# harskish/ganspace

Hardware: NVIDIA H100
Metric: latent samples/sec into PCA (StyleGAN2-ffhq W, N=1e6) (higher is better)
Workload: dtype f32

## Files before the change

ganspace_b200/_native.py:

```python
from __future__ import annotations

import contextlib
import ctypes as C
import os
from pathlib import Path

import torch

_LIB_PATH = Path(__file__).resolve().parent / "libganspace_b200.so"
_lib = None

_P, _I, _L, _Z, _D, _F = C.c_void_p, C.c_int, C.c_int64, C.c_size_t, C.c_double, C.c_float
SIGNATURES = {
    "gsb_abi_version": (_I, []),
    "gsb_last_error": (C.c_char_p, []),
    "gsb_legacy_normal_f32": (_I, [_P, _I, _L, _P, _L, _P]),
    "gsb_legacy_truncnorm_f32": (_I, [_P, _I, _L, _D, _D, _F, _P, _L, _P]),
    "gsb_mt19937_raw_u32": (_I, [_P, _I, _L, _P, _L, _P]),
    "gsb_mt19937_jump_polys": (_I, [_L, _I, _P]),
    "gsb_mt19937_jump_state_host": (_I, [C.c_uint32, _P, _P]),
    "gsb_legacy_normal_split_step_words": (_L, [_L, _I]),
    "gsb_legacy_normal_split_workspace_bytes": (_Z, [_I, _L, _I]),
    "gsb_legacy_normal_f32_split": (_I, [_P, _I, _L, _P, _L, _I, _P, _P, _Z, _P]),
    "gsb_legacy_normal_split_status": (_I, [_P, _I, _L, _I, _P, _P]),
# ... 140 lines not shown
    def add_rows(self, name, n):
        self.rows[name] = self.rows.get(name, 0) + int(n)

    def count(self, n):
        self.launches += n

    class _Sec:
        def __init__(self, outer, name):
            self.o, self.name = outer, name

        def __enter__(self):
            if self.o.timing:
                self.e0 = torch.cuda.Event(enable_timing=True)
                self.e1 = torch.cuda.Event(enable_timing=True)
                self.e0.record(torch.cuda.current_stream())

        def __exit__(self, *a):
            if self.o.timing:
                self.e1.record(torch.cuda.current_stream())
                self.o._events.setdefault(self.name, []).append((self.e0, self.e1))
            self.o.mark(self.name + " done")

    def section(self, name):
        return self._Sec(self, name)

    def section_ms(self):
        torch.cuda.synchronize()
        return {k: (sum(a.elapsed_time(b) for a, b in v), len(v)) for k, v in self._events.items()}


instrument = _Instrument()

SECTION_KERNELS = {
    "mapping": "mapping MLP: pixelnorm_split + 8 x mapping_layer_tc_kernel (wgmma, fp16 hi/lo x3)",
    "linear": "gen_z linear: mapping_layer_tc_kernel (wgmma, fp16 hi/lo x3, bias epilogue, TMA store) for n >= 128",
    "synthesis": "StyledConv chain: tap-GEMM tc_gemm_plain (wgmma) + gather/scatter/blur epilogues",
}


def kernel_name(section: str) -> str:
    if section == "mapping" and os.environ.get("GANSPACE_B200_MAPPING", MAPPING_DEFAULT) == "simt":
        return "mapping MLP: pixelnorm + 8 x sgemm_tn_bias_act_kernel (fp32 FMA)"
    return SECTION_KERNELS.get(section, section)


class _Scratch:

    def __init__(self):
        self._bufs = {}

    def get(self, key, nbytes: int, device) -> torch.Tensor:
        k = (key, str(device))
        buf = self._bufs.get(k)
        if buf is None or buf.numel() < nbytes:
            buf = torch.empty(max(int(nbytes), 256), dtype=torch.uint8, device=device)
            self._bufs[k] = buf
        return buf

    def clear(self):
        self._bufs.clear()


scratch = _Scratch()


_jump_polys = {}


def jump_polys(n_per_stream: int, parts: int, device) -> torch.Tensor:
    import numpy as np
    lib = load()
    step = int(lib.gsb_legacy_normal_split_step_words(int(n_per_stream), int(parts)))
    key = (step, parts - 1)
    if key not in _jump_polys:
        table = np.zeros((parts - 1, 624), np.uint32)
# ... 92 lines not shown
        self.n_layers, self.dim = int(weight.shape[0]), int(weight.shape[1])
        assert weight.shape == (self.n_layers, self.dim, self.dim) and bias.shape == (self.n_layers, self.dim)
        self.device = dev
        self.packed = torch.empty(lib.gsb_mapping_packed_bytes(self.n_layers, self.dim), dtype=torch.uint8, device=dev)
        w = weight.detach().to(dev, torch.float32).contiguous()
        b = bias.detach().to(dev, torch.float32).contiguous()
        with torch.cuda.device(dev):
            _check(lib.gsb_mapping_pack(_ptr(w), _ptr(b), self.n_layers, self.dim, float(lr_mul),
                                        _ptr(self.packed), _stream()), "gsb_mapping_pack")

    def check(self):
        flags = C.c_uint(0)
        with torch.cuda.device(self.device):
            _check(load().gsb_mapping_status(_ptr(self.packed), self.n_layers, self.dim, C.byref(flags)),
                   "gsb_mapping_status")
        if flags.value & 1:
            raise NativeError("mapping network: an activation exceeded fp16 range in the tensor-core path; "
                              "results are invalid (set GANSPACE_B200_MAPPING=simt)")

    def forward(self, z: torch.Tensor, out: torch.Tensor = None, pixelnorm: bool = True,
                force_simt: bool = None, leave_free_sms: int = 0) -> torch.Tensor:
        lib = load()
        if force_simt is None:
            force_simt = os.environ.get("GANSPACE_B200_MAPPING", MAPPING_DEFAULT) == "simt"
        assert z.is_cuda and z.dtype == torch.float32 and z.shape[-1] == self.dim
        z2 = z.reshape(-1, self.dim)
        if not z2.is_contiguous():
            z2 = z2.contiguous()
        n = z2.shape[0]
        if out is None:
            out = torch.empty_like(z2)
        ws_bytes = lib.gsb_mapping_workspace_bytes(n, self.dim)
        ws = scratch.get("mapping", ws_bytes, z.device)
        flags = (1 if pixelnorm else 0) | (2 if force_simt else 0) | ((int(leave_free_sms) & 0xff) << 8)
        with torch.cuda.device(z.device), instrument.section("mapping"):
            _check(lib.gsb_mapping_forward(_ptr(self.packed), self.n_layers, self.dim, _ptr(z2), _ptr(out), n,
                                           flags, _ptr(ws), ws.numel(), _stream()), "gsb_mapping_forward")
        instrument.count(self.n_layers + (1 if pixelnorm else 0))
        instrument.add_rows("mapping", n)
        return out.reshape(z.shape)


def linear(x: torch.Tensor, w: torch.Tensor, bias: torch.Tensor = None, lrelu: bool = False, bounded: bool = False) -> torch.Tensor:
    lib = load()
    assert x.is_cuda and x.dtype == torch.float32 and w.dtype == torch.float32 and x.shape[-1] == w.shape[1]
    x2 = x.reshape(-1, x.shape[-1]).contiguous()
    w = w.contiguous()
    n, K = x2.shape
    N = w.shape[0]
    y = torch.empty((n, N), dtype=torch.float32, device=x.device)
    flags = (1 if lrelu else 0) | (2 if bounded else 0)
    ws = scratch.get("linear", lib.gsb_linear_workspace_bytes(n, N, K, flags), x.device)
    with torch.cuda.device(x.device), instrument.section("linear"):
        _check(lib.gsb_linear_forward(_ptr(x2), _ptr(w), _ptr(bias.contiguous() if bias is not None else None), _ptr(y),
                                      n, N, K, flags, _ptr(ws), ws.numel(), _stream()), "gsb_linear_forward")
    instrument.count(5 if (bounded and n >= 128 and N % 256 == 0 and K % 64 == 0) else 1)
    instrument.add_rows("linear", n)
    return y.reshape(*x.shape[:-1], N)


def mapping_pixelnorm(z: torch.Tensor) -> torch.Tensor:
    lib = load()
    assert z.is_cuda and z.dtype == torch.float32
    dim = z.shape[-1]
    z2 = z.reshape(-1, dim).contiguous()
    out = torch.empty_like(z2)
    ws = scratch.get("mapping", lib.gsb_mapping_workspace_bytes(z2.shape[0], dim), z.device)
    with torch.cuda.device(z.device):
        _check(lib.gsb_mapping_forward(C.c_void_p(0), 0, dim, _ptr(z2), _ptr(out), z2.shape[0], 1, _ptr(ws),
                                       ws.numel(), _stream()), "gsb_mapping_forward")
    return out.reshape(z.shape)
# ... 491 lines not shown
```

ganspace_b200/csrc/mapping.cu:

```cuda
#include "common.cuh"

namespace gsb {

size_t mapping_tc_packed_bytes(int n_layers, int dim);
int mapping_tc_pack(const float *pw, int n_layers, int dim, void *tc_base, cudaStream_t st);
int mapping_forward_tc(const float *pb, void *tc_base, int n_layers, int dim, const float *d_z, float *d_w,
                       int64_t n, bool pixelnorm, void *ws, int leave_free_sms, cudaStream_t st);
size_t mapping_tc_workspace_bytes(int64_t n, int dim);
size_t tc_linear_workspace_bytes(int64_t n, int N, int K);
int tc_linear(const float *x, const float *w, const float *bias, float *y, int64_t n, int N, int K, bool lrelu, void *ws,
              cudaStream_t st);
unsigned *mapping_tc_overflow_flag(void *tc_base, int n_layers, int dim);

static inline size_t simt_packed_bytes(int n_layers, int dim) {
    return align_up(((size_t)n_layers * dim * dim + (size_t)n_layers * dim) * sizeof(float), 256);
}
static inline bool tc_supported(int n_layers, int dim) { return n_layers > 0 && dim % 256 == 0; }

__global__ void mapping_pack_kernel(const float *__restrict__ w, const float *__restrict__ b,
                                    int n_layers, int dim, float scale, float lr_mul,
                                    float *__restrict__ pw, float *__restrict__ pb) {
    int64_t nw = (int64_t)n_layers * dim * dim;
    int64_t nb = (int64_t)n_layers * dim;
    for (int64_t i = blockIdx.x * (int64_t)blockDim.x + threadIdx.x; i < nw + nb;
         i += (int64_t)gridDim.x * blockDim.x) {
        if (i < nw) pw[i] = __fmul_rn(w[i], scale);
        else pb[i - nw] = __fmul_rn(b[i - nw], lr_mul);
    }
}

__global__ void pixelnorm_kernel(const float *__restrict__ x, float *__restrict__ y, int64_t n, int dim) {
    int64_t row = blockIdx.x * (int64_t)(blockDim.x >> 5) + (threadIdx.x >> 5);
    if (row >= n) return;
    const int lane = threadIdx.x & 31;
    const float4 *xr = reinterpret_cast<const float4 *>(x + row * dim);
    float4 *yr = reinterpret_cast<float4 *>(y + row * dim);
    float s = 0.f;
    for (int i = lane; i < dim / 4; i += 32) {
        float4 v = xr[i];
        s += v.x * v.x + v.y * v.y + v.z * v.z + v.w * v.w;
// ... 134 lines not shown
    float scale = (float)((1.0 / sqrt((double)dim)) * (double)lr_mul);
    gsb::mapping_pack_kernel<<<512, 256, 0, (cudaStream_t)stream>>>(d_weight, d_bias, n_layers, dim, scale,
                                                                   lr_mul, pw, pb);
    GSB_CHECK_LAUNCH();
    if (gsb::tc_supported(n_layers, dim)) {
        void *tc_base = reinterpret_cast<char *>(d_packed) + gsb::simt_packed_bytes(n_layers, dim);
        return gsb::mapping_tc_pack(pw, n_layers, dim, tc_base, (cudaStream_t)stream);
    }
    return GSB_OK;
}

extern "C" size_t gsb_mapping_workspace_bytes(int64_t n, int dim) {
    size_t simt = 2 * gsb::align_up((size_t)n * dim * sizeof(float), 256);
    size_t tc = gsb::mapping_tc_workspace_bytes(n, dim);
    return simt > tc ? simt : tc;
}

extern "C" int gsb_mapping_forward(const void *d_packed, int n_layers, int dim, const float *d_z,
                                   float *d_w, int64_t n, int flags, void *d_workspace,
                                   size_t workspace_bytes, gsb_stream_t stream) {
    GSB_CHECK_ARG(d_z && d_w && (d_packed || n_layers == 0), "mapping_forward: null pointer");
    GSB_CHECK_ARG(n_layers >= 0 && dim % 128 == 0, "mapping_forward: dim must be a multiple of 128");
    GSB_CHECK_ARG(n_layers > 0 || (flags & 1), "mapping_forward: nothing to do (n_layers == 0 without PixelNorm)");
    if (n == 0) return GSB_OK;
    if (workspace_bytes < gsb_mapping_workspace_bytes(n, dim) || !d_workspace) {
        gsb::set_error("mapping_forward: workspace too small (%zu < %zu)", workspace_bytes,
                       gsb_mapping_workspace_bytes(n, dim));
        return GSB_ERR_WORKSPACE;
    }
    const float *pw = reinterpret_cast<const float *>(d_packed);
    const float *pb = pw + (size_t)n_layers * dim * dim;
    if (!(flags & 2) && gsb::tc_supported(n_layers, dim)) {
        void *tc_base = reinterpret_cast<char *>(const_cast<void *>(d_packed)) + gsb::simt_packed_bytes(n_layers, dim);
        return gsb::mapping_forward_tc(pb, tc_base, n_layers, dim, d_z, d_w, n, (flags & 1) != 0, d_workspace,
                                       (flags >> 8) & 0xff, (cudaStream_t)stream);
    }
    float *tmp0 = reinterpret_cast<float *>(d_workspace);
    float *tmp1 = reinterpret_cast<float *>(reinterpret_cast<char *>(d_workspace) +
                                            gsb::align_up((size_t)n * dim * sizeof(float), 256));
    return gsb::mapping_forward_simt(pw, pb, n_layers, dim, d_z, d_w, n, (flags & 1) != 0, tmp0, tmp1,
                                     (cudaStream_t)stream);
}

extern "C" int gsb_mapping_status(const void *d_packed, int n_layers, int dim, unsigned *h_flags) {
    GSB_CHECK_ARG(d_packed && h_flags, "mapping_status: null pointer");
    *h_flags = 0;
    if (!gsb::tc_supported(n_layers, dim)) return GSB_OK;
    void *tc_base = reinterpret_cast<char *>(const_cast<void *>(d_packed)) + gsb::simt_packed_bytes(n_layers, dim);
    GSB_CHECK_CUDA(cudaMemcpy(h_flags, gsb::mapping_tc_overflow_flag(tc_base, n_layers, dim), sizeof(unsigned),
                              cudaMemcpyDeviceToHost));
    return GSB_OK;
}

static bool linear_tc_eligible(int64_t n, int N, int K, int flags) {
    return (flags & 2) && n >= 128 && N % 256 == 0 && K % 64 == 0;
}

extern "C" size_t gsb_linear_workspace_bytes(int64_t n, int N, int K, int flags) {
    size_t b = (size_t)N * sizeof(float);
    if (linear_tc_eligible(n, N, K, flags)) {
        size_t t = gsb::tc_linear_workspace_bytes(n, N, K) + gsb::align_up((size_t)N * sizeof(float), 256);
        if (t > b) b = t;
    }
    return b;
}

extern "C" int gsb_linear_forward(const float *d_x, const float *d_w, const float *d_bias, float *d_y, int64_t n,
                                  int N, int K, int flags, void *d_workspace, size_t workspace_bytes,
// ... 27 lines not shown
```

ganspace_b200/csrc/mapping_tc.cu:

```cuda
#include "tc_common.cuh"
#include <stdlib.h>

namespace gsb {

constexpr int TC_BLOCK_M = 128;
constexpr int TC_BLOCK_N = 128;
constexpr int TC_BLOCK_K = 64;
constexpr int TC_STAGES = 3;
constexpr int TC_FRAG_ROWS = 64;
constexpr uint32_t TC_A_BYTES = TC_BLOCK_M * TC_BLOCK_K * 2;
constexpr uint32_t TC_W_BYTES = TC_BLOCK_N * TC_BLOCK_K * 2;
constexpr uint32_t TC_STAGE_BYTES = 2 * TC_A_BYTES + 2 * TC_W_BYTES;
constexpr uint32_t TC_BOX_BYTES = TC_FRAG_ROWS * 128;
constexpr uint32_t TC_STAGING_BYTES = 2 * 2 * TC_BOX_BYTES;
constexpr int TC_THREADS = tc::CONSUMER_THREADS + 128;
constexpr uint32_t TC_SMEM_BYTES = TC_STAGES * TC_STAGE_BYTES + TC_STAGING_BYTES + 64  + 1024 ;
static_assert(TC_SMEM_BYTES <= 232448, "mapping_layer_tc_kernel: shared memory exceeds the H100's 227 KB per block");

struct TcParams {
    const float *bias;
    __half *out_hi;
    __half *out_lo;
    float *out_f32;
    unsigned *overflow;
// ... 128 lines not shown
            int stage = g0 % TC_STAGES, prev = stage;
            uint32_t phase = (uint32_t)(g0 / TC_STAGES) & 1;
            if (i > 0) mbar_wait(&turn_bar[wg], (uint32_t)((i - 1) >> 1) & 1);
            for (int kb = 0; kb < num_k_blocks; ++kb) {
                mbar_wait(&full_bar[stage], phase);
                if (!(p.dbg & 8)) {
                    const uint32_t st = smem_u32(smem + stage * TC_STAGE_BYTES);
                    const uint32_t sw = st + 2 * TC_A_BYTES;
                    const uint64_t d_wh = sw128_kmajor_desc(sw), d_wl = sw128_kmajor_desc(sw + TC_W_BYTES);
                    wgmma_fence();
                    split_kblock_m64n128(acc0, sw128_kmajor_desc(st), sw128_kmajor_desc(st + TC_A_BYTES), d_wh, d_wl, kb > 0);
                    split_kblock_m64n128(acc1, sw128_kmajor_desc(st + TC_A_BYTES / 2),
                                         sw128_kmajor_desc(st + TC_A_BYTES + TC_A_BYTES / 2), d_wh, d_wl, kb > 0);
                    wgmma_commit();
                }
                wgmma_wait_1();
                if (kb > 0 && lane == 0) mbar_arrive(&empty_bar[prev]);
                if (kb == num_k_blocks - 1 && lane == 0) mbar_arrive(&turn_bar[wg ^ 1]);
                prev = stage;
                if (++stage == TC_STAGES) { stage = 0; phase ^= 1; }
            }
            wgmma_wait_all();
            if (lane == 0) mbar_arrive(&empty_bar[prev]);
            store_chunk(acc0, 0, m0, n0, 0);
            store_chunk(acc0, 32, m0, n0, 64);
            store_chunk(acc1, 0, m0 + TC_FRAG_ROWS, n0, 0);
            store_chunk(acc1, 32, m0 + TC_FRAG_ROWS, n0, 64);
        }
        if (ovf) atomicOr(p.overflow, 1u);
        if (storer) asm volatile("cp.async.bulk.wait_group 0;" ::: "memory");
    }
}

__global__ void pixelnorm_split_kernel(const float *__restrict__ x, __half *__restrict__ hi, __half *__restrict__ lo,
                                       int64_t n, int dim, int do_norm, unsigned *overflow) {
    int64_t row = blockIdx.x * (int64_t)(blockDim.x >> 5) + (threadIdx.x >> 5);
    if (row >= n) return;
    const int lane = threadIdx.x & 31;
    const float4 *xr = reinterpret_cast<const float4 *>(x + row * dim);
    float r = 1.f;
    if (do_norm) {
        float s = 0.f;
        for (int i = lane; i < dim / 4; i += 32) {
            float4 v = xr[i];
            s += v.x * v.x + v.y * v.y + v.z * v.z + v.w * v.w;
        }
        s = warp_sum(s);
        r = 1.0f / sqrtf(s / (float)dim + 1e-8f);
    }
    bool ovf = false;
    for (int i = lane; i < dim / 4; i += 32) {
        float4 v = xr[i];
        float f[4] = {v.x * r, v.y * r, v.z * r, v.w * r};
        __half h[4], l[4];
#pragma unroll
        for (int q = 0; q < 4; ++q) {
            h[q] = __float2half_rn(f[q]);
            l[q] = __float2half_rn(f[q] - __half2float(h[q]));
            ovf |= fabsf(f[q]) > 60000.f;
        }
        uint2 ph, pl;
        ph.x = (uint32_t)__half_as_ushort(h[0]) | ((uint32_t)__half_as_ushort(h[1]) << 16);
        ph.y = (uint32_t)__half_as_ushort(h[2]) | ((uint32_t)__half_as_ushort(h[3]) << 16);
        pl.x = (uint32_t)__half_as_ushort(l[0]) | ((uint32_t)__half_as_ushort(l[1]) << 16);
        pl.y = (uint32_t)__half_as_ushort(l[2]) | ((uint32_t)__half_as_ushort(l[3]) << 16);
        reinterpret_cast<uint2 *>(hi + row * dim)[i] = ph;
// ... 24 lines not shown
    }
}

__global__ void absmax_kernel(const float *__restrict__ x, int64_t count, float *__restrict__ out) {
    float m = 0.f;
    for (int64_t i = blockIdx.x * (int64_t)blockDim.x + threadIdx.x; i < count; i += (int64_t)gridDim.x * blockDim.x)
        m = fmaxf(m, fabsf(x[i]));
    for (int o = 16; o > 0; o >>= 1) m = fmaxf(m, __shfl_xor_sync(0xffffffffu, m, o));
    if ((threadIdx.x & 31) == 0) atomicMax(reinterpret_cast<int *>(out), __float_as_int(m));
}

static int make_tmap_f16(CUtensorMap *map, const void *base, uint64_t rows, uint64_t cols, uint32_t box_rows) {
    const uint64_t dims[2] = {cols, rows};
    const uint64_t strides[1] = {cols * 2};
    const uint32_t box[2] = {(uint32_t)TC_BLOCK_K, box_rows};
    return tc_make_tmap_f16(map, base, 2, dims, strides, box);
}

static int make_tmap_f32_out(CUtensorMap *map, const void *base, uint64_t rows, uint64_t cols) {
    TcEncodeTiledFn enc = tc_encode_fn();
    if (!enc) { set_error("cuTensorMapEncodeTiled entry point not available"); return GSB_ERR_CUDA; }
    cuuint64_t gdim[2] = {cols, rows};
    cuuint64_t gstride[1] = {cols * 4};
    cuuint32_t box[2] = {32, (cuuint32_t)TC_FRAG_ROWS};
    cuuint32_t estr[2] = {1, 1};
    CUresult r = enc(map, CU_TENSOR_MAP_DATA_TYPE_FLOAT32, 2, const_cast<void *>(base), gdim, gstride, box, estr,
                     CU_TENSOR_MAP_INTERLEAVE_NONE, CU_TENSOR_MAP_SWIZZLE_128B, CU_TENSOR_MAP_L2_PROMOTION_L2_256B,
                     CU_TENSOR_MAP_FLOAT_OOB_FILL_NONE);
    if (r != CUDA_SUCCESS) { set_error("cuTensorMapEncodeTiled (fp32 output) failed (%d)", (int)r); return GSB_ERR_CUDA; }
    return GSB_OK;
}

size_t mapping_tc_packed_bytes(int n_layers, int dim) {
    return align_up((size_t)n_layers * dim * dim * 2, 256) * 2 + align_up((size_t)3 * n_layers * sizeof(float), 256) + 256;
}

struct TcPackView {
    __half *w_hi, *w_lo;
    float *inv_wscale, *wscale, *absmax;
    unsigned *overflow;
};
static TcPackView tc_pack_view(void *base, int n_layers, int dim) {
    TcPackView v;
    char *p = reinterpret_cast<char *>(base);
    size_t wb = align_up((size_t)n_layers * dim * dim * 2, 256);
    v.w_hi = reinterpret_cast<__half *>(p);
    v.w_lo = reinterpret_cast<__half *>(p + wb);
    v.inv_wscale = reinterpret_cast<float *>(p + 2 * wb);
    v.wscale = v.inv_wscale + n_layers;
    v.absmax = v.wscale + n_layers;
    v.overflow = reinterpret_cast<unsigned *>(p + 2 * wb + align_up((size_t)3 * n_layers * sizeof(float), 256));
    return v;
}

int mapping_tc_pack(const float *pw, int n_layers, int dim, void *tc_base, cudaStream_t st) {
    TcPackView v = tc_pack_view(tc_base, n_layers, dim);
    GSB_CHECK_CUDA(cudaMemsetAsync(v.inv_wscale, 0, (size_t)3 * n_layers * sizeof(float), st));
    GSB_CHECK_CUDA(cudaMemsetAsync(v.overflow, 0, sizeof(unsigned), st));
    const int64_t per = (int64_t)dim * dim;
    for (int l = 0; l < n_layers; ++l) {
        absmax_kernel<<<64, 256, 0, st>>>(pw + l * per, per, v.absmax + l);
        GSB_CHECK_LAUNCH();
        pick_wscale_kernel<<<1, 1, 0, st>>>(v.absmax + l, v.wscale + l, v.inv_wscale + l);
        GSB_CHECK_LAUNCH();
        weight_split_kernel<<<256, 256, 0, st>>>(pw + l * per, per, v.wscale + l, v.w_hi + l * per, v.w_lo + l * per);
        GSB_CHECK_LAUNCH();
    }
    return GSB_OK;
}

static int tc_ensure_attr() {
    static bool attr_set = false;
    if (!attr_set) {
        GSB_CHECK_CUDA(cudaFuncSetAttribute(mapping_layer_tc_kernel, cudaFuncAttributeMaxDynamicSharedMemorySize, (int)TC_SMEM_BYTES));
        attr_set = true;
    }
    return GSB_OK;
}

static int tc_launch_layer(const CUtensorMap &tm_ah, const CUtensorMap &tm_al, const CUtensorMap &tm_wh, const CUtensorMap &tm_wl,
                           TcParams p, int leave_free_sms, cudaStream_t st) {
    CUtensorMap tm_o0, tm_o1;
    if (p.out_f32) {
        if (int r = make_tmap_f32_out(&tm_o0, p.out_f32, (uint64_t)p.M, (uint64_t)p.N_total)) return r;
        tm_o1 = tm_o0;
    } else {
        if (int r = make_tmap_f16(&tm_o0, p.out_hi, (uint64_t)p.M, (uint64_t)p.N_total, TC_FRAG_ROWS)) return r;
        if (int r = make_tmap_f16(&tm_o1, p.out_lo, (uint64_t)p.M, (uint64_t)p.N_total, TC_FRAG_ROWS)) return r;
    }
    const int m_tiles = (p.M + TC_BLOCK_M - 1) / TC_BLOCK_M, n_tiles = (p.N_total + TC_BLOCK_N - 1) / TC_BLOCK_N;
    int avail = num_sms() - leave_free_sms;
    if (avail < 16) avail = 16;
    if (avail > num_sms()) avail = num_sms();
    {
        static int dbg = -1;
        if (dbg < 0) { const char *e = getenv("GANSPACE_B200_MAPPING_DBG"); dbg = e ? atoi(e) : 0; }
        p.dbg = dbg;
    }
    const int64_t units = (int64_t)m_tiles * n_tiles;
    const int grid = units < avail ? (int)units : avail;
    mapping_layer_tc_kernel<<<grid, TC_THREADS, TC_SMEM_BYTES, st>>>(tm_ah, tm_al, tm_wh, tm_wl, tm_o0, tm_o1, p);
    GSB_CHECK_LAUNCH();
    return GSB_OK;
}

int tc_gemm_plain(const __half *a_hi, const __half *a_lo, int64_t M, int K, const __half *w_hi, const __half *w_lo, int N,
                  const float *inv_wscale, float *out, unsigned *overflow, int leave_free_sms, cudaStream_t st) {
    GSB_CHECK_ARG(N % 32 == 0 && N >= 32 && K % 8 == 0 && K >= 8 && M > 0 && M < (1ll << 31),
                  "tc_gemm_plain: need N%%32==0, K%%8==0 (M=%lld N=%d K=%d)", (long long)M, N, K);
    if (int r = tc_ensure_attr()) return r;
    CUtensorMap tm_ah, tm_al, tm_wh, tm_wl;
    if (int r = make_tmap_f16(&tm_ah, a_hi, (uint64_t)M, (uint64_t)K, TC_BLOCK_M)) return r;
    if (int r = make_tmap_f16(&tm_al, a_lo, (uint64_t)M, (uint64_t)K, TC_BLOCK_M)) return r;
    if (int r = make_tmap_f16(&tm_wh, w_hi, (uint64_t)N, (uint64_t)K, TC_BLOCK_N)) return r;
    if (int r = make_tmap_f16(&tm_wl, w_lo, (uint64_t)N, (uint64_t)K, TC_BLOCK_N)) return r;
    TcParams p;
    p.bias = nullptr; p.out_hi = nullptr; p.out_lo = nullptr; p.out_f32 = out; p.overflow = overflow;
    p.inv_wscale = inv_wscale; p.M = (int)M; p.N_total = N; p.K = K; p.mode = 1;
    return tc_launch_layer(tm_ah, tm_al, tm_wh, tm_wl, p, leave_free_sms, st);
}

size_t tc_linear_workspace_bytes(int64_t n, int N, int K) {
    return 2 * align_up((size_t)n * K * 2, 256) + 2 * align_up((size_t)N * K * 2, 256) + 512;
}

int tc_linear(const float *x, const float *w, const float *bias, float *y, int64_t n, int N, int K, bool lrelu, void *ws,
              cudaStream_t st) {
    GSB_CHECK_ARG(N % 256 == 0 && K % TC_BLOCK_K == 0 && n > 0 && n < (1ll << 31) && bias, "tc_linear: need N%%256==0, K%%64==0, bias");
    if (int r = tc_ensure_attr()) return r;
    char *p0 = reinterpret_cast<char *>(ws);
    const size_t xb = align_up((size_t)n * K * 2, 256), wb = align_up((size_t)N * K * 2, 256);
    __half *x_hi = (__half *)p0, *x_lo = (__half *)(p0 + xb), *w_hi = (__half *)(p0 + 2 * xb), *w_lo = (__half *)(p0 + 2 * xb + wb);
    float *scal = (float *)(p0 + 2 * xb + 2 * wb);
    unsigned *overflow = (unsigned *)(p0 + 2 * xb + 2 * wb + 256);
    GSB_CHECK_CUDA(cudaMemsetAsync(scal, 0, 512, st));
    absmax_kernel<<<256, 256, 0, st>>>(w, (int64_t)N * K, scal + 2);
    GSB_CHECK_LAUNCH();
    pick_wscale_kernel<<<1, 1, 0, st>>>(scal + 2, scal + 1, scal);
    GSB_CHECK_LAUNCH();
    weight_split_kernel<<<1024, 256, 0, st>>>(w, (int64_t)N * K, scal + 1, w_hi, w_lo);
    GSB_CHECK_LAUNCH();
    pixelnorm_split_kernel<<<(unsigned)((n + 7) / 8), 256, 0, st>>>(x, x_hi, x_lo, n, K, 0, overflow);
    GSB_CHECK_LAUNCH();
    CUtensorMap tm_ah, tm_al, tm_wh, tm_wl;
    if (int r = make_tmap_f16(&tm_ah, x_hi, (uint64_t)n, (uint64_t)K, TC_BLOCK_M)) return r;
    if (int r = make_tmap_f16(&tm_al, x_lo, (uint64_t)n, (uint64_t)K, TC_BLOCK_M)) return r;
    if (int r = make_tmap_f16(&tm_wh, w_hi, (uint64_t)N, (uint64_t)K, TC_BLOCK_N)) return r;
    if (int r = make_tmap_f16(&tm_wl, w_lo, (uint64_t)N, (uint64_t)K, TC_BLOCK_N)) return r;
    TcParams p;
    p.bias = bias; p.out_hi = nullptr; p.out_lo = nullptr; p.out_f32 = y; p.overflow = overflow;
    p.inv_wscale = scal; p.M = (int)n; p.N_total = N; p.K = K; p.mode = lrelu ? 0 : 2;
    return tc_launch_layer(tm_ah, tm_al, tm_wh, tm_wl, p, 0, st);
}

int mapping_forward_tc(const float *pb, void *tc_base, int n_layers, int dim,
                       const float *d_z, float *d_w, int64_t n, bool pixelnorm, void *ws, int leave_free_sms,
                       cudaStream_t st) {
    GSB_CHECK_ARG(dim % 256 == 0 && dim % TC_BLOCK_K == 0, "mapping_forward_tc: dim must be a multiple of 256");
    GSB_CHECK_ARG(n < (1ll << 31), "mapping_forward_tc: too many rows");
    TcPackView v = tc_pack_view(tc_base, n_layers, dim);
    const size_t buf = align_up((size_t)n * dim * 2, 256);
    __half *a_hi[2] = {reinterpret_cast<__half *>(ws), reinterpret_cast<__half *>((char *)ws + 2 * buf)};
    __half *a_lo[2] = {reinterpret_cast<__half *>((char *)ws + buf), reinterpret_cast<__half *>((char *)ws + 3 * buf)};

    if (int r = tc_ensure_attr()) return r;
    pixelnorm_split_kernel<<<(unsigned)((n + 7) / 8), 256, 0, st>>>(d_z, a_hi[0], a_lo[0], n, dim, pixelnorm ? 1 : 0,
                                                                  v.overflow);
    GSB_CHECK_LAUNCH();
    const int64_t per = (int64_t)dim * dim;
    for (int l = 0; l < n_layers; ++l) {
        const int src = l & 1, dst = src ^ 1;
        CUtensorMap tm_ah, tm_al, tm_wh, tm_wl;
        if (int r = make_tmap_f16(&tm_ah, a_hi[src], (uint64_t)n, dim, TC_BLOCK_M)) return r;
        if (int r = make_tmap_f16(&tm_al, a_lo[src], (uint64_t)n, dim, TC_BLOCK_M)) return r;
        if (int r = make_tmap_f16(&tm_wh, v.w_hi + l * per, dim, dim, TC_BLOCK_N)) return r;
        if (int r = make_tmap_f16(&tm_wl, v.w_lo + l * per, dim, dim, TC_BLOCK_N)) return r;
        TcParams p;
        p.bias = pb + (int64_t)l * dim;
        const bool last = (l == n_layers - 1);
        p.out_hi = last ? nullptr : a_hi[dst];
        p.out_lo = last ? nullptr : a_lo[dst];
        p.out_f32 = last ? d_w : nullptr;
        p.overflow = v.overflow;
        p.inv_wscale = v.inv_wscale + l;
        p.M = (int)n; p.N_total = dim; p.K = dim; p.mode = 0;
        if (int r = tc_launch_layer(tm_ah, tm_al, tm_wh, tm_wl, p, leave_free_sms, st)) return r;
    }
    return GSB_OK;
}

size_t mapping_tc_workspace_bytes(int64_t n, int dim) { return 4 * align_up((size_t)n * dim * 2, 256); }

unsigned *mapping_tc_overflow_flag(void *tc_base, int n_layers, int dim) {
    return tc_pack_view(tc_base, n_layers, dim).overflow;
}

}
```

ganspace_b200/csrc/tc_common.cuh:

```cuda
#pragma once
#include "common.cuh"
#include <cuda.h>
#include <cuda_fp16.h>

namespace gsb {
namespace tc {

constexpr int CONSUMER_THREADS = 256;
constexpr int THREADS = CONSUMER_THREADS + 32;
constexpr int PRODUCER_WARP = CONSUMER_THREADS / 32;

__device__ __forceinline__ uint32_t smem_u32(const void *p) { return (uint32_t)__cvta_generic_to_shared(p); }

__device__ __forceinline__ void mbar_init(uint64_t *bar, uint32_t count) {
    asm volatile("mbarrier.init.shared::cta.b64 [%0], %1;" ::"r"(smem_u32(bar)), "r"(count));
}
__device__ __forceinline__ void mbar_fence_init() { asm volatile("fence.mbarrier_init.release.cluster;" ::: "memory"); }
__device__ __forceinline__ void mbar_wait(uint64_t *bar, uint32_t parity) {
    asm volatile(
        "{\n\t"
        ".reg .pred P1;\n\t"
        "TCW_LOOP:\n\t"
        "mbarrier.try_wait.parity.shared::cta.b64 P1, [%0], %1, 0x989680;\n\t"
        "@P1 bra TCW_DONE;\n\t"
        "bra TCW_LOOP;\n\t"
        "TCW_DONE:\n\t"
        "}" ::"r"(smem_u32(bar)), "r"(parity)
        : "memory");
}
__device__ __forceinline__ void mbar_arrive(uint64_t *bar) {
    asm volatile("mbarrier.arrive.shared::cta.b64 _, [%0];" ::"r"(smem_u32(bar)) : "memory");
}
__device__ __forceinline__ void mbar_arrive_expect_tx(uint64_t *bar, uint32_t bytes) {
    asm volatile("mbarrier.arrive.expect_tx.shared::cta.b64 _, [%0], %1;" ::"r"(smem_u32(bar)), "r"(bytes) : "memory");
}

__device__ __forceinline__ void tma_prefetch_desc(const CUtensorMap *map) {
    asm volatile("prefetch.tensormap [%0];" ::"l"(map) : "memory");
}
__device__ __forceinline__ void tma_load_2d(const CUtensorMap *map, uint64_t *bar, void *dst, int c0, int c1) {
    asm volatile(
        "cp.async.bulk.tensor.2d.shared::cluster.global.mbarrier::complete_tx::bytes [%0], [%1, {%3, %4}], [%2];"
        ::"r"(smem_u32(dst)), "l"(map), "r"(smem_u32(bar)), "r"(c0), "r"(c1)
        : "memory");
}
__device__ __forceinline__ void tma_load_3d(const CUtensorMap *map, uint64_t *bar, void *dst, int c0, int c1, int c2) {
    asm volatile(
        "cp.async.bulk.tensor.3d.shared::cluster.global.mbarrier::complete_tx::bytes [%0], [%1, {%3, %4, %5}], [%2];"
        ::"r"(smem_u32(dst)), "l"(map), "r"(smem_u32(bar)), "r"(c0), "r"(c1), "r"(c2)
        : "memory");
}
__device__ __forceinline__ void tma_store_2d(const CUtensorMap *map, const void *src, int c0, int c1) {
    asm volatile("cp.async.bulk.tensor.2d.global.shared::cta.bulk_group [%0, {%2, %3}], [%1];"
                 ::"l"(map), "r"(smem_u32(src)), "r"(c0), "r"(c1) : "memory");
}

__device__ __forceinline__ void wgmma_fence() { asm volatile("wgmma.fence.sync.aligned;" ::: "memory"); }
__device__ __forceinline__ void wgmma_commit() { asm volatile("wgmma.commit_group.sync.aligned;" ::: "memory"); }
__device__ __forceinline__ void wgmma_wait_all() { asm volatile("wgmma.wait_group.sync.aligned 0;" ::: "memory"); }
__device__ __forceinline__ void wgmma_wait_1() { asm volatile("wgmma.wait_group.sync.aligned 1;" ::: "memory"); }

__device__ __forceinline__ uint64_t sw128_kmajor_desc(uint32_t smem_addr) {
    uint64_t d = 0;
    d |= (uint64_t)((smem_addr & 0x3FFFF) >> 4);
    d |= (uint64_t)1 << 16;
    d |= (uint64_t)(1024 >> 4) << 32;
    d |= (uint64_t)1 << 62;
    return d;
}

__device__ __forceinline__ void wgmma_m64n128(float (&d)[64], uint64_t da, uint64_t db, uint32_t accumulate) {
    asm volatile(
        "{\n\t"
        ".reg .pred p;\n\t"
        "setp.ne.b32 p, %66, 0;\n\t"
        "wgmma.mma_async.sync.aligned.m64n128k16.f32.f16.f16 "
        "{%0, %1, %2, %3, %4, %5, %6, %7, %8, %9, %10, %11, %12, %13, %14, %15, "
        "%16, %17, %18, %19, %20, %21, %22, %23, %24, %25, %26, %27, %28, %29, %30, %31, "
        "%32, %33, %34, %35, %36, %37, %38, %39, %40, %41, %42, %43, %44, %45, %46, %47, "
        "%48, %49, %50, %51, %52, %53, %54, %55, %56, %57, %58, %59, %60, %61, %62, %63}, "
        "%64, %65, p, 1, 1, 0, 0;\n\t"
        "}"
        : "+f"(d[0]), "+f"(d[1]), "+f"(d[2]), "+f"(d[3]), "+f"(d[4]), "+f"(d[5]), "+f"(d[6]), "+f"(d[7]),
          "+f"(d[8]), "+f"(d[9]), "+f"(d[10]), "+f"(d[11]), "+f"(d[12]), "+f"(d[13]), "+f"(d[14]), "+f"(d[15]),
          "+f"(d[16]), "+f"(d[17]), "+f"(d[18]), "+f"(d[19]), "+f"(d[20]), "+f"(d[21]), "+f"(d[22]), "+f"(d[23]),
          "+f"(d[24]), "+f"(d[25]), "+f"(d[26]), "+f"(d[27]), "+f"(d[28]), "+f"(d[29]), "+f"(d[30]), "+f"(d[31]),
          "+f"(d[32]), "+f"(d[33]), "+f"(d[34]), "+f"(d[35]), "+f"(d[36]), "+f"(d[37]), "+f"(d[38]), "+f"(d[39]),
          "+f"(d[40]), "+f"(d[41]), "+f"(d[42]), "+f"(d[43]), "+f"(d[44]), "+f"(d[45]), "+f"(d[46]), "+f"(d[47]),
          "+f"(d[48]), "+f"(d[49]), "+f"(d[50]), "+f"(d[51]), "+f"(d[52]), "+f"(d[53]), "+f"(d[54]), "+f"(d[55]),
          "+f"(d[56]), "+f"(d[57]), "+f"(d[58]), "+f"(d[59]), "+f"(d[60]), "+f"(d[61]), "+f"(d[62]), "+f"(d[63])
        : "l"(da), "l"(db), "r"(accumulate)
        : "memory");
}

__device__ __forceinline__ void split_kblock_m64n128(float (&d)[64], uint64_t ah, uint64_t al, uint64_t bh, uint64_t bl,
                                                     bool accumulate) {
#pragma unroll
    for (int k = 0; k < 4; ++k) {
        const uint64_t koff = (uint64_t)(2 * k);
        wgmma_m64n128(d, ah + koff, bh + koff, (accumulate || k > 0) ? 1u : 0u);
// ... 23 lines not shown
```

Measured before the change: 18.33 million.

## Fuse all eight mapping MLP layers into one persistent wgmma kernel

Adds a persistent warp-specialized kernel that keeps a 64-row activation tile resident in shared memory across all mapping layers. Weights are prepacked into per-k-step stage buffers and streamed through a 3-stage TMA bulk-load ring, so intermediate activations no longer round-trip through global memory between eight separate launches. The old per-layer path stays available through an environment setting. In exchange the packed weight buffer doubles in size and each tile re-streams the full weight set, so throughput depends on L2 holding the roughly 8 MB of staged weights.

```diff
diff --git a/ganspace_b200/_native.py b/ganspace_b200/_native.py
--- a/ganspace_b200/_native.py
+++ b/ganspace_b200/_native.py
@@ -196,15 +196,18 @@
 instrument = _Instrument()
 
 SECTION_KERNELS = {
-    "mapping": "mapping MLP: pixelnorm_split + 8 x mapping_layer_tc_kernel (wgmma, fp16 hi/lo x3)",
+    "mapping": "mapping MLP: pixelnorm_split + mapping_mlp_fused_tc_kernel (8 layers in one launch, wgmma, fp16 hi/lo x3)",
     "linear": "gen_z linear: mapping_layer_tc_kernel (wgmma, fp16 hi/lo x3, bias epilogue, TMA store) for n >= 128",
     "synthesis": "StyledConv chain: tap-GEMM tc_gemm_plain (wgmma) + gather/scatter/blur epilogues",
 }
 
 
 def kernel_name(section: str) -> str:
-    if section == "mapping" and os.environ.get("GANSPACE_B200_MAPPING", MAPPING_DEFAULT) == "simt":
+    mapping = os.environ.get("GANSPACE_B200_MAPPING", MAPPING_DEFAULT)
+    if section == "mapping" and mapping == "simt":
         return "mapping MLP: pixelnorm + 8 x sgemm_tn_bias_act_kernel (fp32 FMA)"
+    if section == "mapping" and mapping == "layers":
+        return "mapping MLP: pixelnorm_split + 8 x mapping_layer_tc_kernel (wgmma, fp16 hi/lo x3)"
     return SECTION_KERNELS.get(section, section)
 
 
@@ -363,11 +366,13 @@
             out = torch.empty_like(z2)
         ws_bytes = lib.gsb_mapping_workspace_bytes(n, self.dim)
         ws = scratch.get("mapping", ws_bytes, z.device)
-        flags = (1 if pixelnorm else 0) | (2 if force_simt else 0) | ((int(leave_free_sms) & 0xff) << 8)
+        per_layer = os.environ.get("GANSPACE_B200_MAPPING", MAPPING_DEFAULT) == "layers"
+        flags = (1 if pixelnorm else 0) | (2 if force_simt else 0) | (4 if per_layer else 0) | ((int(leave_free_sms) & 0xff) << 8)
         with torch.cuda.device(z.device), instrument.section("mapping"):
             _check(lib.gsb_mapping_forward(_ptr(self.packed), self.n_layers, self.dim, _ptr(z2), _ptr(out), n,
                                            flags, _ptr(ws), ws.numel(), _stream()), "gsb_mapping_forward")
-        instrument.count(self.n_layers + (1 if pixelnorm else 0))
+        fused = self.dim == 512 and not force_simt and not per_layer
+        instrument.count((1 if fused else self.n_layers) + (1 if pixelnorm else 0))
         instrument.add_rows("mapping", n)
         return out.reshape(z.shape)
 
diff --git a/ganspace_b200/csrc/mapping.cu b/ganspace_b200/csrc/mapping.cu
--- a/ganspace_b200/csrc/mapping.cu
+++ b/ganspace_b200/csrc/mapping.cu
@@ -5,7 +5,7 @@
 size_t mapping_tc_packed_bytes(int n_layers, int dim);
 int mapping_tc_pack(const float *pw, int n_layers, int dim, void *tc_base, cudaStream_t st);
 int mapping_forward_tc(const float *pb, void *tc_base, int n_layers, int dim, const float *d_z, float *d_w,
-                       int64_t n, bool pixelnorm, void *ws, int leave_free_sms, cudaStream_t st);
+                       int64_t n, bool pixelnorm, bool per_layer, void *ws, int leave_free_sms, cudaStream_t st);
 size_t mapping_tc_workspace_bytes(int64_t n, int dim);
 size_t tc_linear_workspace_bytes(int64_t n, int N, int K);
 int tc_linear(const float *x, const float *w, const float *bias, float *y, int64_t n, int N, int K, bool lrelu, void *ws,
@@ -206,8 +206,8 @@
     const float *pb = pw + (size_t)n_layers * dim * dim;
     if (!(flags & 2) && gsb::tc_supported(n_layers, dim)) {
         void *tc_base = reinterpret_cast<char *>(const_cast<void *>(d_packed)) + gsb::simt_packed_bytes(n_layers, dim);
-        return gsb::mapping_forward_tc(pb, tc_base, n_layers, dim, d_z, d_w, n, (flags & 1) != 0, d_workspace,
-                                       (flags >> 8) & 0xff, (cudaStream_t)stream);
+        return gsb::mapping_forward_tc(pb, tc_base, n_layers, dim, d_z, d_w, n, (flags & 1) != 0, (flags & 4) != 0,
+                                       d_workspace, (flags >> 8) & 0xff, (cudaStream_t)stream);
     }
     float *tmp0 = reinterpret_cast<float *>(d_workspace);
     float *tmp1 = reinterpret_cast<float *>(reinterpret_cast<char *>(d_workspace) +
diff --git a/ganspace_b200/csrc/mapping_tc.cu b/ganspace_b200/csrc/mapping_tc.cu
--- a/ganspace_b200/csrc/mapping_tc.cu
+++ b/ganspace_b200/csrc/mapping_tc.cu
@@ -184,6 +184,183 @@
     }
 }
 
+constexpr int FU_DIM = 512;
+constexpr int FU_ROWS = 64;
+constexpr int FU_KSTEPS = FU_DIM / 16;
+constexpr int FU_KBLOCKS = FU_DIM / 64;
+constexpr uint32_t FU_BOX_BYTES = FU_ROWS * 128;
+constexpr uint32_t FU_ACT_BYTES = 2 * FU_KBLOCKS * FU_BOX_BYTES;
+constexpr uint32_t FU_WPLANE_BYTES = FU_DIM * 16 * 2;
+constexpr uint32_t FU_STAGE_BYTES = 2 * FU_WPLANE_BYTES;
+constexpr int FU_STAGES = 3;
+constexpr uint32_t FU_SMEM_BYTES = FU_ACT_BYTES + FU_STAGES * FU_STAGE_BYTES + 64  + 1024 ;
+static_assert(FU_SMEM_BYTES <= 232448, "mapping_mlp_fused_tc_kernel: shared memory exceeds the H100's 227 KB per block");
+
+struct FusedParams {
+    const float *bias;
+    const uint8_t *w_stages;
+    const float *inv_wscale;
+    unsigned *overflow;
+    int M, n_layers;
+    int dbg;
+};
+
+__global__ void __launch_bounds__(TC_THREADS, 1)
+mapping_mlp_fused_tc_kernel(const __grid_constant__ CUtensorMap tm_in_hi, const __grid_constant__ CUtensorMap tm_in_lo,
+                            const __grid_constant__ CUtensorMap tm_out, const FusedParams p) {
+    using namespace tc;
+    extern __shared__ uint8_t smem_raw[];
+    uint8_t *act = reinterpret_cast<uint8_t *>((reinterpret_cast<uintptr_t>(smem_raw) + 1023) & ~(uintptr_t)1023);
+    uint8_t *ring = act + FU_ACT_BYTES;
+    uint64_t *bars = reinterpret_cast<uint64_t *>(ring + FU_STAGES * FU_STAGE_BYTES);
+    uint64_t *full_bar = bars;
+    uint64_t *empty_bar = bars + FU_STAGES;
+    uint64_t *act_full = bars + 2 * FU_STAGES;
+    uint64_t *act_empty = bars + 2 * FU_STAGES + 1;
+
+    const int warp = threadIdx.x >> 5, lane = threadIdx.x & 31;
+    const int num_tiles = (p.M + FU_ROWS - 1) / FU_ROWS;
+
+    if (threadIdx.x == 0) {
+        for (int s = 0; s < FU_STAGES; ++s) { mbar_init(&full_bar[s], 1); mbar_init(&empty_bar[s], 8); }
+        mbar_init(act_full, 1); mbar_init(act_empty, 2);
+        mbar_fence_init();
+    }
+    if (warp == PRODUCER_WARP && lane == 0) {
+        tma_prefetch_desc(&tm_in_hi); tma_prefetch_desc(&tm_in_lo); tma_prefetch_desc(&tm_out);
+    }
+    __syncthreads();
+
+    if (warp >= PRODUCER_WARP) {
+        asm volatile("setmaxnreg.dec.sync.aligned.u32 40;");
+        if (warp == PRODUCER_WARP && lane == 0) {
+            int stage = 0; uint32_t phase = 0;
+            for (int t = blockIdx.x; t < num_tiles; t += gridDim.x) {
+                for (int l = 0; l < p.n_layers; ++l) {
+                    for (int s = 0; s < FU_KSTEPS; ++s) {
+                        mbar_wait(&empty_bar[stage], phase ^ 1);
+                        mbar_arrive_expect_tx(&full_bar[stage], (p.dbg & 2) ? 0u : FU_STAGE_BYTES);
+                        if (!(p.dbg & 2))
+                            bulk_load_1d(ring + stage * FU_STAGE_BYTES,
+                                         p.w_stages + ((size_t)l * FU_KSTEPS + s) * FU_STAGE_BYTES, FU_STAGE_BYTES, &full_bar[stage]);
+                        if (++stage == FU_STAGES) { stage = 0; phase ^= 1; }
+                    }
+                }
+            }
+        } else if (warp == PRODUCER_WARP + 1 && lane == 0) {
+            uint32_t j = 0;
+            for (int t = blockIdx.x; t < num_tiles; t += gridDim.x, ++j) {
+                mbar_wait(act_empty, (j & 1) ^ 1);
+                mbar_arrive_expect_tx(act_full, FU_ACT_BYTES);
+                for (int kb = 0; kb < FU_KBLOCKS; ++kb) {
+                    tma_load_2d(&tm_in_hi, act_full, act + kb * FU_BOX_BYTES, kb * 64, t * FU_ROWS);
+                    tma_load_2d(&tm_in_lo, act_full, act + (FU_KBLOCKS + kb) * FU_BOX_BYTES, kb * 64, t * FU_ROWS);
+                }
+            }
+        }
+    } else {
+        asm volatile("setmaxnreg.inc.sync.aligned.u32 232;");
+        const int wg = warp >> 2;
+        const int rr0 = (warp & 3) * 16 + (lane >> 2);
+        const int q2 = 2 * (lane & 3);
+        const float slope = 0.2f, gain = 1.41421356237309515f;
+        const bool storer = ((threadIdx.x & 127) == 0);
+        const uint32_t act_u = smem_u32(act), ring_u = smem_u32(ring);
+        bool ovf = false;
+        float acc0[64], acc1[64];
+#pragma unroll
+        for (int j = 0; j < 64; ++j) { acc0[j] = 0.f; acc1[j] = 0.f; }
+
+        auto epilogue = [&](const float (&acc)[64], const int q, const bool last, const float inv_wscale, const float *bias) {
+#pragma unroll
+            for (int g = 0; g < 16; ++g) {
+                const int col = 256 * wg + 128 * q + 8 * g + q2;
+                const float2 b = __ldg(reinterpret_cast<const float2 *>(bias + col));
+#pragma unroll
+                for (int h = 0; h < 2; ++h) {
+                    const int rr = rr0 + 8 * h;
+                    float f[2];
+#pragma unroll
+                    for (int e = 0; e < 2; ++e) {
+                        float x = __fmul_rn(acc[4 * g + 2 * h + e], inv_wscale) + (e ? b.y : b.x);
+                        x = (x >= 0.f) ? x : __fmul_rn(x, slope);
+                        f[e] = __fmul_rn(gain, x);
+                    }
+                    const uint32_t sw = (uint32_t)(rr & 7);
+                    if (last) {
+                        const int cb = col & 31;
+                        *reinterpret_cast<float2 *>(act + (col >> 5) * FU_BOX_BYTES + rr * 128 + ((((uint32_t)cb >> 2) ^ sw) << 4) +
+                                                    (cb & 3) * 4) = make_float2(f[0], f[1]);
+                    } else {
+                        uint32_t hi, lo;
+                        split2(f[0], f[1], hi, lo);
+                        ovf |= (fabsf(f[0]) > 60000.f) | (fabsf(f[1]) > 60000.f);
+                        uint8_t *row = act + (col >> 6) * FU_BOX_BYTES + rr * 128 + ((((uint32_t)g & 7) ^ sw) << 4) + 2 * q2;
+                        *reinterpret_cast<uint32_t *>(row) = hi;
+                        *reinterpret_cast<uint32_t *>(row + FU_KBLOCKS * FU_BOX_BYTES) = lo;
+                    }
+                }
+            }
+        };
+
+        int stage = 0; uint32_t phase = 0;
+        uint32_t j = 0;
+        for (int t = blockIdx.x; t < num_tiles; t += gridDim.x, ++j) {
+            mbar_wait(act_full, j & 1);
+            for (int l = 0; l < p.n_layers; ++l) {
+                int prev = stage;
+                for (int s = 0; s < FU_KSTEPS; ++s) {
+                    mbar_wait(&full_bar[stage], phase);
+                    if (!(p.dbg & 8)) {
+                        const uint32_t a = act_u + (s >> 2) * FU_BOX_BYTES;
+                        const uint64_t koff = (uint64_t)(2 * (s & 3));
+                        const uint64_t d_ah = sw128_kmajor_desc(a) + koff;
+                        const uint64_t d_al = sw128_kmajor_desc(a + FU_KBLOCKS * FU_BOX_BYTES) + koff;
+                        const uint32_t w = ring_u + stage * FU_STAGE_BYTES + wg * 8192;
+                        wgmma_fence();
+                        const uint64_t d_wh0 = core_kmajor_desc(w, 128, 256), d_wl0 = core_kmajor_desc(w + FU_WPLANE_BYTES, 128, 256);
+                        wgmma_m64n128(acc0, d_ah, d_wh0, s > 0 ? 1u : 0u);
+                        wgmma_m64n128(acc0, d_al, d_wh0, 1u);
+                        wgmma_m64n128(acc0, d_ah, d_wl0, 1u);
+                        const uint64_t d_wh1 = core_kmajor_desc(w + 4096, 128, 256),
+                                       d_wl1 = core_kmajor_desc(w + FU_WPLANE_BYTES + 4096, 128, 256);
+                        wgmma_m64n128(acc1, d_ah, d_wh1, s > 0 ? 1u : 0u);
+                        wgmma_m64n128(acc1, d_al, d_wh1, 1u);
+                        wgmma_m64n128(acc1, d_ah, d_wl1, 1u);
+                        wgmma_commit();
+                    }
+                    wgmma_wait_1();
+                    if (s > 0 && lane == 0) mbar_arrive(&empty_bar[prev]);
+                    prev = stage;
+                    if (++stage == FU_STAGES) { stage = 0; phase ^= 1; }
+                }
+                wgmma_wait_all();
+                if (lane == 0) mbar_arrive(&empty_bar[prev]);
+                asm volatile("bar.sync 1, 256;" ::: "memory");
+                const bool last = (l == p.n_layers - 1);
+                const float inv_wscale = __ldg(p.inv_wscale + l);
+                const float *bias = p.bias + (size_t)l * FU_DIM;
+                epilogue(acc0, 0, last, inv_wscale, bias);
+                epilogue(acc1, 1, last, inv_wscale, bias);
+                asm volatile("fence.proxy.async.shared::cta;" ::: "memory");
+                if (!last) asm volatile("bar.sync 1, 256;" ::: "memory");
+            }
+            asm volatile("bar.sync %0, 128;" ::"r"(2 + wg) : "memory");
+            if (storer) {
+                if (!(p.dbg & 1)) {
+#pragma unroll 1
+                    for (int b = 8 * wg; b < 8 * wg + 8; ++b) tma_store_2d(&tm_out, act + b * FU_BOX_BYTES, 32 * b, t * FU_ROWS);
+                }
+                asm volatile("cp.async.bulk.commit_group;" ::: "memory");
+                asm volatile("cp.async.bulk.wait_group.read 0;" ::: "memory");
+                mbar_arrive(act_empty);
+            }
+        }
+        if (ovf) atomicOr(p.overflow, 1u);
+        if (storer) asm volatile("cp.async.bulk.wait_group 0;" ::: "memory");
+    }
+}
+
 __global__ void pixelnorm_split_kernel(const float *__restrict__ x, __half *__restrict__ hi, __half *__restrict__ lo,
                                        int64_t n, int dim, int do_norm, unsigned *overflow) {
     int64_t row = blockIdx.x * (int64_t)(blockDim.x >> 5) + (threadIdx.x >> 5);
@@ -274,11 +451,12 @@
 }
 
 size_t mapping_tc_packed_bytes(int n_layers, int dim) {
-    return align_up((size_t)n_layers * dim * dim * 2, 256) * 2 + align_up((size_t)3 * n_layers * sizeof(float), 256) + 256;
+    return align_up((size_t)n_layers * dim * dim * 2, 256) * 4 + align_up((size_t)3 * n_layers * sizeof(float), 256) + 256;
 }
 
 struct TcPackView {
     __half *w_hi, *w_lo;
+    __half *w_stages;
     float *inv_wscale, *wscale, *absmax;
     unsigned *overflow;
 };
@@ -288,11 +466,25 @@
     size_t wb = align_up((size_t)n_layers * dim * dim * 2, 256);
     v.w_hi = reinterpret_cast<__half *>(p);
     v.w_lo = reinterpret_cast<__half *>(p + wb);
-    v.inv_wscale = reinterpret_cast<float *>(p + 2 * wb);
+    v.w_stages = reinterpret_cast<__half *>(p + 2 * wb);
+    v.inv_wscale = reinterpret_cast<float *>(p + 4 * wb);
     v.wscale = v.inv_wscale + n_layers;
     v.absmax = v.wscale + n_layers;
-    v.overflow = reinterpret_cast<unsigned *>(p + 2 * wb + align_up((size_t)3 * n_layers * sizeof(float), 256));
+    v.overflow = reinterpret_cast<unsigned *>(p + 4 * wb + align_up((size_t)3 * n_layers * sizeof(float), 256));
     return v;
+}
+
+__global__ void weight_stage_kernel(const __half *__restrict__ hi, const __half *__restrict__ lo, int dim, int64_t count,
+                                    __half *__restrict__ stages) {
+    const int64_t per = (int64_t)dim * dim;
+    for (int64_t i = blockIdx.x * (int64_t)blockDim.x + threadIdx.x; i < count; i += (int64_t)gridDim.x * blockDim.x) {
+        const int64_t l = i / per;
+        const int n = (int)((i % per) / dim), k = (int)(i % dim);
+        const int kk = k & 15;
+        const int64_t o = (l * (dim / 16) + (k >> 4)) * (2 * 16 * dim) + (n >> 3) * 128 + (kk >> 3) * 64 + (n & 7) * 8 + (kk & 7);
+        stages[o] = hi[i];
+        stages[o + 16 * dim] = lo[i];
+    }
 }
 
 int mapping_tc_pack(const float *pw, int n_layers, int dim, void *tc_base, cudaStream_t st) {
@@ -308,6 +500,8 @@
         weight_split_kernel<<<256, 256, 0, st>>>(pw + l * per, per, v.wscale + l, v.w_hi + l * per, v.w_lo + l * per);
         GSB_CHECK_LAUNCH();
     }
+    weight_stage_kernel<<<256, 256, 0, st>>>(v.w_hi, v.w_lo, dim, n_layers * per, v.w_stages);
+    GSB_CHECK_LAUNCH();
     return GSB_OK;
 }
 
@@ -315,9 +509,23 @@
     static bool attr_set = false;
     if (!attr_set) {
         GSB_CHECK_CUDA(cudaFuncSetAttribute(mapping_layer_tc_kernel, cudaFuncAttributeMaxDynamicSharedMemorySize, (int)TC_SMEM_BYTES));
+        GSB_CHECK_CUDA(cudaFuncSetAttribute(mapping_mlp_fused_tc_kernel, cudaFuncAttributeMaxDynamicSharedMemorySize, (int)FU_SMEM_BYTES));
         attr_set = true;
     }
     return GSB_OK;
+}
+
+static int persistent_grid(int64_t units, int leave_free_sms) {
+    int avail = num_sms() - leave_free_sms;
+    if (avail < 16) avail = 16;
+    if (avail > num_sms()) avail = num_sms();
+    return units < avail ? (int)units : avail;
+}
+
+static int mapping_dbg() {
+    static int dbg = -1;
+    if (dbg < 0) { const char *e = getenv("GANSPACE_B200_MAPPING_DBG"); dbg = e ? atoi(e) : 0; }
+    return dbg;
 }
 
 static int tc_launch_layer(const CUtensorMap &tm_ah, const CUtensorMap &tm_al, const CUtensorMap &tm_wh, const CUtensorMap &tm_wl,
@@ -331,16 +539,8 @@
         if (int r = make_tmap_f16(&tm_o1, p.out_lo, (uint64_t)p.M, (uint64_t)p.N_total, TC_FRAG_ROWS)) return r;
     }
     const int m_tiles = (p.M + TC_BLOCK_M - 1) / TC_BLOCK_M, n_tiles = (p.N_total + TC_BLOCK_N - 1) / TC_BLOCK_N;
-    int avail = num_sms() - leave_free_sms;
-    if (avail < 16) avail = 16;
-    if (avail > num_sms()) avail = num_sms();
-    {
-        static int dbg = -1;
-        if (dbg < 0) { const char *e = getenv("GANSPACE_B200_MAPPING_DBG"); dbg = e ? atoi(e) : 0; }
-        p.dbg = dbg;
-    }
-    const int64_t units = (int64_t)m_tiles * n_tiles;
-    const int grid = units < avail ? (int)units : avail;
+    p.dbg = mapping_dbg();
+    const int grid = persistent_grid((int64_t)m_tiles * n_tiles, leave_free_sms);
     mapping_layer_tc_kernel<<<grid, TC_THREADS, TC_SMEM_BYTES, st>>>(tm_ah, tm_al, tm_wh, tm_wl, tm_o0, tm_o1, p);
     GSB_CHECK_LAUNCH();
     return GSB_OK;
@@ -396,7 +596,7 @@
 }
 
 int mapping_forward_tc(const float *pb, void *tc_base, int n_layers, int dim,
-                       const float *d_z, float *d_w, int64_t n, bool pixelnorm, void *ws, int leave_free_sms,
+                       const float *d_z, float *d_w, int64_t n, bool pixelnorm, bool per_layer, void *ws, int leave_free_sms,
                        cudaStream_t st) {
     GSB_CHECK_ARG(dim % 256 == 0 && dim % TC_BLOCK_K == 0, "mapping_forward_tc: dim must be a multiple of 256");
     GSB_CHECK_ARG(n < (1ll << 31), "mapping_forward_tc: too many rows");
@@ -409,6 +609,19 @@
     pixelnorm_split_kernel<<<(unsigned)((n + 7) / 8), 256, 0, st>>>(d_z, a_hi[0], a_lo[0], n, dim, pixelnorm ? 1 : 0,
                                                                   v.overflow);
     GSB_CHECK_LAUNCH();
+    if (dim == FU_DIM && !per_layer) {
+        CUtensorMap tm_in_hi, tm_in_lo, tm_out;
+        if (int r = make_tmap_f16(&tm_in_hi, a_hi[0], (uint64_t)n, dim, FU_ROWS)) return r;
+        if (int r = make_tmap_f16(&tm_in_lo, a_lo[0], (uint64_t)n, dim, FU_ROWS)) return r;
+        if (int r = make_tmap_f32_out(&tm_out, d_w, (uint64_t)n, dim)) return r;
+        FusedParams p;
+        p.bias = pb; p.w_stages = reinterpret_cast<const uint8_t *>(v.w_stages); p.inv_wscale = v.inv_wscale;
+        p.overflow = v.overflow; p.M = (int)n; p.n_layers = n_layers; p.dbg = mapping_dbg();
+        const int grid = persistent_grid((n + FU_ROWS - 1) / FU_ROWS, leave_free_sms);
+        mapping_mlp_fused_tc_kernel<<<grid, TC_THREADS, FU_SMEM_BYTES, st>>>(tm_in_hi, tm_in_lo, tm_out, p);
+        GSB_CHECK_LAUNCH();
+        return GSB_OK;
+    }
     const int64_t per = (int64_t)dim * dim;
     for (int l = 0; l < n_layers; ++l) {
         const int src = l & 1, dst = src ^ 1;
diff --git a/ganspace_b200/csrc/tc_common.cuh b/ganspace_b200/csrc/tc_common.cuh
--- a/ganspace_b200/csrc/tc_common.cuh
+++ b/ganspace_b200/csrc/tc_common.cuh
@@ -54,6 +54,10 @@
     asm volatile("cp.async.bulk.tensor.2d.global.shared::cta.bulk_group [%0, {%2, %3}], [%1];"
                  ::"l"(map), "r"(smem_u32(src)), "r"(c0), "r"(c1) : "memory");
 }
+__device__ __forceinline__ void bulk_load_1d(void *dst, const void *src, uint32_t bytes, uint64_t *bar) {
+    asm volatile("cp.async.bulk.shared::cluster.global.mbarrier::complete_tx::bytes [%0], [%1], %2, [%3];"
+                 ::"r"(smem_u32(dst)), "l"(src), "r"(bytes), "r"(smem_u32(bar)) : "memory");
+}
 
 __device__ __forceinline__ void wgmma_fence() { asm volatile("wgmma.fence.sync.aligned;" ::: "memory"); }
 __device__ __forceinline__ void wgmma_commit() { asm volatile("wgmma.commit_group.sync.aligned;" ::: "memory"); }
@@ -66,6 +70,14 @@
     d |= (uint64_t)1 << 16;
     d |= (uint64_t)(1024 >> 4) << 32;
     d |= (uint64_t)1 << 62;
+    return d;
+}
+
+__device__ __forceinline__ uint64_t core_kmajor_desc(uint32_t smem_addr, uint32_t lbo, uint32_t sbo) {
+    uint64_t d = 0;
+    d |= (uint64_t)((smem_addr & 0x3FFFF) >> 4);
+    d |= (uint64_t)((lbo >> 4) & 0x3FFF) << 16;
+    d |= (uint64_t)((sbo >> 4) & 0x3FFF) << 32;
     return d;
 }
 
```

New measurement: 17.76 million (median of 6 runs). 3.1% lower.
